# ExaScience/elprep

Measured on AMD Instinct MI355X. Metric: Mreads/s through sort+markdup+BQSR, 150bp PE, higher is better.
Workload: dtype u8/int32/int64 (integer path; float64 finalize on host)

## Files before the change

elprep_amd/csrc/common.hpp:

```cpp
#pragma once

#include <hip/hip_runtime.h>

#include <sched.h>

#include <cstdarg>
#include <cstdint>
#include <cstdio>
#include <cstring>
#include <map>
#include <mutex>
#include <string>
#include <vector>

#include "../../include/elprep_hip.h"
#include "../../include/elprep_hip_debug.h"
#include "derived.hpp"

namespace elp {

constexpr int WAVE = 64;

enum : uint16_t {
  F_MULTIPLE = 0x1, F_PROPER = 0x2, F_UNMAPPED = 0x4, F_NEXT_UNMAPPED = 0x8, F_REVERSED = 0x10, F_NEXT_REVERSED = 0x20,
// ... 116 lines not shown
  int tables_max_cycle = 0;
  unsigned long long tables_quals[2] = {0, 0};
  elp::DVec<unsigned long long> tables_pack;
  elp::DVec<uint8_t> lut_rows_dev;
  void *comm = nullptr;
  bool comm_borrowed = false;
  int (*xport)(void *, int64_t *, size_t) = nullptr;
  void *xport_user = nullptr;
  int (*p2p)(void *, int, const void *, size_t, int, void *, size_t) = nullptr;
  void *p2p_user = nullptr;
  int group_rank = 0, group_world = 1;
  elp_ctx *group_owner = nullptr;
  std::vector<elp_ctx *> group_borrowers;

  elp::DVec<uint8_t> raw;
  elp::DVec<uint64_t> raw_off;
  uint64_t raw_n = 0, raw_bytes = 0;
  uint64_t max_raw_rec = 0;
  elp::DVec<uint8_t> rg_ids;
  elp::DVec<uint32_t> rg_ids_off;
  bool have_rg_ids = false;
  static constexpr size_t TAG_WORDS = 65536 / 32;
  bool tag_filter = false;
  std::vector<uint32_t> h_tag_drop;
  elp::DVec<uint32_t> tag_drop;
  bool replace_rg = false;
  std::string replace_rg_id;
  elp::DVec<uint8_t> replace_rg_dev;
  hipStream_t copy_stream = nullptr;
  elp::DVec<uint8_t> lut_dev;
  void *lut_pinned = nullptr;
  size_t lut_pinned_cap = 0;
  hipEvent_t lut_ev = nullptr;
  hipEvent_t apply_ev = nullptr;
  int lut_uploaded_cycle = 0;
  elp::DVec<uint32_t> lut_wk;
  bool dict_ready = false;
  bool dict_per_cov = false;
  int dict_qlo = 0, dict_nqi = 0, dict_lmax = 0, dict_cycle = 0, dict_ncov = 0;
  hipEvent_t tables_ev = nullptr;
  void *bounce[2] = {nullptr, nullptr};
  hipEvent_t bounce_ev[2] = {nullptr, nullptr};

  uint32_t *mail = nullptr;
  hipEvent_t mail_ev = nullptr;

  elp_ctx *side[2] = {nullptr, nullptr};
  hipEvent_t side_ev[2] = {nullptr, nullptr};
  hipEvent_t side_done[2] = {nullptr, nullptr};
  bool sort_ahead = false;
  uint64_t presort_n = 0;
  uint64_t *presort_ks = nullptr;
  int presort_idx_bits = 0;

  elp::DVec<uint16_t> snap_flag;
  elp::DVec<uint8_t> snap_qual;
  uint64_t snap_n = 0, snap_qual_bytes = 0;

  struct Tuning {
    int count_kernel = 0;
    int apply_kernel = 0;
    int count3_rlog = -1;
    int qual_hint = 0;
    int qual_hint_drop = -1;
    int pair_table_slots = 1 << 20;
    long long bgzf_piece = 1ll << 30;
    int bgzf_weak_guess = 0;
    int score_kernel = 0;
    int mate_path = 0;
    int radix_tile = 0;
    int sort_pairs = 0;
    int tie_rounds = 0;
    int exchange_piece = 0;
    int emit_pass = 0;
    long long bgzf_inflate_piece = 2ll << 30;
    int bgzf_copy_chunk = 0;
    int bgzf_tok_lds = 0;
    int bgzf_first_chunk_div = 4;
    int bgzf_fixed = 0;
    int bgzf_tok_fail_above = 0;
    int bgzf_stored = 0;
    int apply_wgs = 0;
    int count3_grid = 0;
    int presort_tile = 0;
    int side_priority = 0;
  } tune;

  elp::DVec<uint8_t> scratch[8];

  bool profiling = false;
  const char *prof_prefix = nullptr;
  std::vector<std::string> prof_names;
  std::map<std::string, int> prof_index;
  std::vector<uint64_t> prof_launches;
  std::vector<double> prof_ms;
  std::vector<elp::ProfPending> prof_pending;
};

namespace elp {

int set_error(elp_ctx *c, int code, const char *fmt, ...);
int prof_begin(elp_ctx *c, const char *name);
void prof_end(elp_ctx *c, int pending);
int prof_flush(elp_ctx *c);
struct ProfScope {
  elp_ctx *c;
  const char *saved;
  ProfScope(elp_ctx *ctx, const char *prefix) : c(ctx), saved(ctx->prof_prefix) { ctx->prof_prefix = prefix; }
  ~ProfScope() { c->prof_prefix = saved; }
};

#define ELP_HIP(ctx, call)                                                                             \
  do {                                                                                                 \
    hipError_t e__ = (call);                                                                           \
    if (e__ != hipSuccess)                                                                             \
      return elp::set_error((ctx), e__ == hipErrorOutOfMemory ? ELP_ERR_NOMEM : ELP_ERR_HIP, "%s failed: %s (%s:%d)", #call, \
                            hipGetErrorString(e__), __FILE__, __LINE__);                               \
  } while (0)

#define ELP_TRY(expr)            \
  do {                           \
    int rc__ = (expr);           \
    if (rc__ != 0) return rc__;  \
  } while (0)

bool sync_spin();
inline void spin_relax(unsigned &spins) {
  if (++spins < 4096u) {
#if defined(__x86_64__) || defined(__i386__)
    __builtin_ia32_pause();
#elif defined(__aarch64__)
    asm volatile("yield");
#endif
  } else {
    sched_yield();
  }
}
inline hipError_t stream_wait(hipStream_t st) {
  if (!sync_spin()) return hipStreamSynchronize(st);
  hipError_t e;
  unsigned spins = 0;
  while ((e = hipStreamQuery(st)) == hipErrorNotReady) spin_relax(spins);
  return e;
}
inline hipError_t event_wait(hipEvent_t ev) {
  if (!sync_spin()) return hipEventSynchronize(ev);
  hipError_t e;
  unsigned spins = 0;
  while ((e = hipEventQuery(ev)) == hipErrorNotReady) spin_relax(spins);
  return e;
}

int debug_poison();
bool debug_trace();

template <class T>
int ensure(elp_ctx *c, DVec<T> &v, size_t n, bool keep = false, size_t keep_elems = 0) {
  if (n <= v.cap) return 0;
  size_t ncap = keep ? (n + n / 2 + 16) : n;
  T *np = nullptr;
  ELP_HIP(c, hipMalloc((void **)&np, ncap * sizeof(T) + debug_guard_bytes()));
  if (debug_guard_bytes()) debug_guard_arm(np, ncap * sizeof(T));
  if (const int pz = debug_poison(); pz >= 0) {
    ELP_HIP(c, hipMemsetAsync(np, pz, ncap * sizeof(T), c->stream));
    ELP_HIP(c, elp::stream_wait(c->stream));
  }
// ... 135 lines not shown
```

elprep_amd/csrc/ctx.hip:

```cpp
#include "common.hpp"

namespace elp {

namespace {
constexpr size_t GUARD = 4096;
constexpr uint8_t GUARD_BYTE = 0xC3;
std::mutex guard_mu;
std::map<void *, size_t> guard_of;
int guard_check_one(void *p, size_t payload) {
  uint8_t host[GUARD];
  if (hipDeviceSynchronize() != hipSuccess || hipMemcpy(host, static_cast<uint8_t *>(p) + payload, GUARD, hipMemcpyDeviceToHost) != hipSuccess) return 0;
  for (size_t k = 0; k < GUARD; k++)
    if (host[k] != GUARD_BYTE) {
      fprintf(stderr, "[elp] ELP_DEBUG_GUARD: byte %zu behind the end of a %zu-byte device buffer was overwritten (0x%02x)\n", k, payload, host[k]);
      return 1;
    }
  return 0;
}
}
size_t debug_guard_bytes() {
  static const size_t v = [] { const char *e = getenv("ELP_DEBUG_GUARD"); return (e && *e && *e != '0') ? GUARD : (size_t)0; }();
  return v;
}
void debug_guard_arm(void *p, size_t payload) {
// ... 513 lines not shown

int elp_get_permutation(elp_ctx *c, uint32_t *out) {
  if (!c || (!out && c->n)) return ELP_ERR_ARG;
  if (!c->derived.sorted) return set_error(c, ELP_ERR_ARG, "elp_get_permutation: call elp_sort_coordinate or elp_sort_queryname first");
  ELP_TRY(radix_check(c));
  return d2h(c, out, c->perm.p, c->n * sizeof(uint32_t));
}
int elp_get_flags(elp_ctx *c, uint16_t *out) {
  if (!c || (!out && c->n)) return ELP_ERR_ARG;
  ELP_TRY(radix_check(c));
  return d2h(c, out, c->flag.p, c->n * sizeof(uint16_t));
}
int elp_get_adapted(elp_ctx *c, int32_t *upos, int32_t *score) {
  if (!c) return ELP_ERR_ARG;
  ELP_TRY(ensure_adapted(c));
  if (upos) ELP_TRY(d2h(c, upos, c->upos.p, c->n * sizeof(int32_t)));
  if (score) ELP_TRY(d2h(c, score, c->score.p, c->n * sizeof(int32_t)));
  return 0;
}
int elp_get_qual(elp_ctx *c, uint8_t *out) {
  if (!c || (!out && c->qual_bytes)) return ELP_ERR_ARG;
  return d2h(c, out, c->qual.p, c->qual_bytes);
}

int elp_snapshot(elp_ctx *c) {
  if (!c) return ELP_ERR_ARG;
  ELP_HIP(c, hipSetDevice(c->device));
  ELP_TRY(ensure(c, c->snap_flag, c->n + 1));
  ELP_TRY(ensure(c, c->snap_qual, c->qual_bytes + 16));
  if (c->n) ELP_HIP(c, hipMemcpyAsync(c->snap_flag.p, c->flag.p, c->n * sizeof(uint16_t), hipMemcpyDeviceToDevice, c->stream));
  if (c->qual_bytes) ELP_HIP(c, hipMemcpyAsync(c->snap_qual.p, c->qual.p, c->qual_bytes, hipMemcpyDeviceToDevice, c->stream));
  c->snap_n = c->n;
  c->snap_qual_bytes = c->qual_bytes;
  c->derived.have_snapshot = true;
  return 0;
}
int elp_rollback(elp_ctx *c) {
  if (!c) return ELP_ERR_ARG;
  if (!c->derived.have_snapshot || c->snap_n != c->n || c->snap_qual_bytes != c->qual_bytes)
    return set_error(c, ELP_ERR_ARG, "elp_rollback: no snapshot of the current record set");
  ELP_HIP(c, hipSetDevice(c->device));
  if (c->n) ELP_HIP(c, hipMemcpyAsync(c->flag.p, c->snap_flag.p, c->n * sizeof(uint16_t), hipMemcpyDeviceToDevice, c->stream));
  if (c->qual_bytes) ELP_HIP(c, hipMemcpyAsync(c->qual.p, c->snap_qual.p, c->qual_bytes, hipMemcpyDeviceToDevice, c->stream));
  c->derived.flag_qual_restored();
  return 0;
}

int elp_set_tuning(elp_ctx *c, const char *key, int64_t value) {
  if (!c || !key) return ELP_ERR_ARG;
  const std::string k(key);
  const int v = (int)value;
  if (k == "count_kernel") c->tune.count_kernel = v;
  else if (k == "apply_kernel") c->tune.apply_kernel = v;
  else if (k == "bgzf_piece") { if (value < 1) return set_error(c, ELP_ERR_ARG, "elp_set_tuning: bgzf_piece must be positive"); c->tune.bgzf_piece = value; }
  else if (k == "bgzf_weak_guess") c->tune.bgzf_weak_guess = v;
  else if (k == "score_kernel") { c->tune.score_kernel = v; c->derived.score_tuning_changed(); }
  else if (k == "count3_rlog") c->tune.count3_rlog = v;
  else if (k == "qual_hint") { c->tune.qual_hint = v; c->derived.hint_tuning_changed(); }
  else if (k == "qual_hint_drop") { c->tune.qual_hint_drop = v; c->derived.hint_tuning_changed(); }
  else if (k == "pair_table_slots") {
    if (v == 0) { c->tune.pair_table_slots = 1 << 20; return 0; }
    if (v < 2 || v > (1 << 20) || (v & (v - 1))) return set_error(c, ELP_ERR_ARG, "elp_set_tuning: pair_table_slots must be a power of two >= 2");
    c->tune.pair_table_slots = v;
  } else if (k == "mate_path") {
    if (value != 0 && value != 2) return set_error(c, ELP_ERR_ARG, "elp_set_tuning: mate_path is 0 (the library decides) or 2 (every candidate through the table)");
    c->tune.mate_path = v;
  } else if (k == "tie_rounds") c->tune.tie_rounds = v;
  else if (k == "radix_tile") c->tune.radix_tile = v;
  else if (k == "sort_pairs") c->tune.sort_pairs = v;
  else if (k == "exchange_piece") c->tune.exchange_piece = v;
  else if (k == "emit_pass") c->tune.emit_pass = v;
  else if (k == "bgzf_stored") c->tune.bgzf_stored = v;
  else if (k == "bgzf_tok_fail_above") c->tune.bgzf_tok_fail_above = v;
  else if (k == "bgzf_fixed") c->tune.bgzf_fixed = v;
  else if (k == "bgzf_first_chunk_div") c->tune.bgzf_first_chunk_div = v;
  else if (k == "bgzf_tok_lds") c->tune.bgzf_tok_lds = v;
  else if (k == "bgzf_copy_chunk") c->tune.bgzf_copy_chunk = v;
  else if (k == "bgzf_inflate_piece") { if (value < 1) return set_error(c, ELP_ERR_ARG, "elp_set_tuning: bgzf_inflate_piece must be positive"); c->tune.bgzf_inflate_piece = value; }
  else if (k == "md_fused" || k == "bgzf_inflate") {
    if (value != 0) return set_error(c, ELP_ERR_ARG, "elp_set_tuning: key '%s' is retired (only 0 is accepted)", key);
  } else if (k == "apply_wgs") c->tune.apply_wgs = v;
  else if (k == "presort_tile") c->tune.presort_tile = v;
  else if (k == "count3_grid") { if (value < 0) return set_error(c, ELP_ERR_ARG, "elp_set_tuning: count3_grid must not be negative"); c->tune.count3_grid = v; }
  else if (k == "side_priority") c->tune.side_priority = v;
  else return set_error(c, ELP_ERR_ARG, "elp_set_tuning: unknown key '%s'", key);
  return 0;
}

int elp_profile_enable(elp_ctx *c, int on) {
  if (!c) return ELP_ERR_ARG;
  if (!on) { ELP_TRY(prof_flush(c)); prof_merge_side(c); }
  c->profiling = on != 0;
  for (int lane = 0; lane < 2; lane++)
    if (c->side[lane]) c->side[lane]->profiling = c->profiling;
  return 0;
}
int elp_profile_reset(elp_ctx *c) {
  if (!c) return ELP_ERR_ARG;
  ELP_TRY(prof_flush(c));
  prof_merge_side(c);
  for (auto &v : c->prof_launches) v = 0;
  for (auto &v : c->prof_ms) v = 0.0;
  return 0;
}
int elp_profile_count(elp_ctx *c) {
  if (!c) return ELP_ERR_ARG;
  if (prof_flush(c) != 0) return ELP_ERR_HIP;
  prof_merge_side(c);
  return (int)c->prof_names.size();
}
int elp_profile_get(elp_ctx *c, int index, const char **name, uint64_t *launches, double *total_ms) {
  if (!c || index < 0 || index >= (int)c->prof_names.size()) return ELP_ERR_ARG;
  if (name) *name = c->prof_names[index].c_str();
  if (launches) *launches = c->prof_launches[index];
  if (total_ms) *total_ms = c->prof_ms[index];
  return 0;
}

}
```

elprep_amd/csrc/markdup.hip:

```cpp
#include "common.hpp"

namespace elp {

constexpr uint32_t EMPTY = 0xFFFFFFFFu;
constexpr unsigned long long PB_EMPTY = ~0ull;

struct MdCols {
  uint64_t n;
  const int32_t *refid;
  const uint16_t *flag_in;
  const uint16_t *rgid;
  const uint16_t *rg_lib;
  const uint16_t *split;
  const int32_t *upos, *score;
  const uint64_t *qname_off;
  const uint8_t *qname;
};

__device__ __forceinline__ bool is_candidate(uint16_t f) { return (f & (F_UNMAPPED | F_SECONDARY | F_SUPPLEMENTARY)) == 0; }
__device__ __forceinline__ bool is_true_pair(uint16_t f) { return (f & (F_MULTIPLE | F_NEXT_UNMAPPED)) == F_MULTIPLE; }
__device__ __forceinline__ uint16_t lib_of(const MdCols &m, uint32_t i) {
  const uint16_t rg = m.rgid[i];
  return rg == ELP_NIL16 ? (uint16_t)ELP_NIL16 : m.rg_lib[rg];
}
__device__ __forceinline__ uint32_t ld_agent(const uint32_t *p) { return __hip_atomic_load(p, __ATOMIC_RELAXED, __HIP_MEMORY_SCOPE_AGENT); }
__device__ __forceinline__ unsigned long long ld_agent64(const unsigned long long *p) {
  return __hip_atomic_load(p, __ATOMIC_RELAXED, __HIP_MEMORY_SCOPE_AGENT);
}

__device__ __forceinline__ bool key_eq(const uint4 &a, const uint4 &b) { return a.x == b.x && a.y == b.y && a.z == b.z && a.w == b.w; }
__device__ __forceinline__ uint64_t frag_hash(const uint4 &k) {
  const uint64_t h = ((uint64_t)k.x << 32) | k.y;
  return mix64(mix64(h) ^ (((uint64_t)k.w << 32) | (uint64_t)k.z));
}

template <class Eq>
__device__ __forceinline__ uint32_t find_or_insert(uint32_t *table, uint64_t mask, uint64_t h, uint32_t i, Eq eq, uint64_t limit = ~0ull) {
  uint64_t s = h & mask;
  for (uint64_t probes = 0;; probes++) {
    if (probes > limit) return EMPTY;
    const uint32_t cur = atomicCAS(&table[s], EMPTY, i);
    if (cur == EMPTY) return i;
    if (cur == i || eq(cur, i)) return cur;
    s = (s + 1) & mask;
  }
}

__global__ __launch_bounds__(256) void k_frag_insert(MdCols m, const uint4 *__restrict__ fkey, const uint32_t *__restrict__ flist, uint32_t nf,
                                                     uint32_t *table, uint64_t mask, uint32_t *__restrict__ frep, unsigned long long *fbest) {
  const uint32_t j = blockIdx.x * blockDim.x + threadIdx.x;
  if (j >= nf) return;
  const uint32_t i = flist[j];
  const uint4 mine = fkey[i];
  const uint32_t rep = find_or_insert(table, mask, frag_hash(mine), i, [&](uint32_t a, uint32_t) { return key_eq(fkey[a], mine); });
  frep[i] = rep;
  atomicMax(&fbest[rep], (unsigned long long)(uint32_t)m.score[i]);
}
__global__ __launch_bounds__(256) void k_frag_bits(const uint32_t *__restrict__ table, uint64_t nwords, uint32_t *__restrict__ bits) {
  const uint64_t w = (uint64_t)blockIdx.x * blockDim.x + threadIdx.x;
  if (w >= nwords) return;
  const uint4 *t = reinterpret_cast<const uint4 *>(table + 32 * w);
  uint32_t b = 0;
#pragma unroll
  for (int k = 0; k < 8; k++) {
    const uint4 v = t[k];
    b |= (v.x != EMPTY ? 1u : 0u) << (4 * k) | (v.y != EMPTY ? 2u : 0u) << (4 * k) | (v.z != EMPTY ? 4u : 0u) << (4 * k) | (v.w != EMPTY ? 8u : 0u) << (4 * k);
  }
  bits[w] = b;
}
__device__ __forceinline__ void tournament(const MdCols &m, uint32_t *winner, uint32_t me) {
  uint32_t w = ld_agent(winner);
  for (;;) {
    if (w == EMPTY) {
      const uint32_t old = atomicCAS(winner, EMPTY, me);
      if (old == EMPTY) return;
      w = old;
      continue;
    }
    const int cq = qname_cmp(m.qname, m.qname_off, me, w);
    const bool better = cq < 0 || (cq == 0 && me > w);
    if (!better) return;
    const uint32_t old = atomicCAS(winner, w, me);
    if (old == w) return;
    w = old;
  }
}

__global__ __launch_bounds__(256) void k_frag_tie(MdCols m, const uint32_t *__restrict__ flist, uint32_t nf, const uint32_t *__restrict__ frep,
                                                  const unsigned long long *__restrict__ fbest, uint32_t *fwinner) {
  const uint32_t j = blockIdx.x * blockDim.x + threadIdx.x;
  if (j >= nf) return;
  const uint32_t i = flist[j];
  const uint32_t rep = frep[i];
  const unsigned long long b = fbest[rep];
  if ((b >> 63) || (unsigned long long)(uint32_t)m.score[i] != b) return;
  tournament(m, &fwinner[rep], (uint32_t)i);
}

__global__ __launch_bounds__(256) void k_frag_flag(MdCols m, const uint32_t *__restrict__ flist, uint32_t nf, const uint32_t *__restrict__ frep,
                                                   const unsigned long long *__restrict__ fbest, const uint32_t *__restrict__ fwinner,
                                                   uint16_t *__restrict__ flag_out) {
  const uint32_t j = blockIdx.x * blockDim.x + threadIdx.x;
  if (j >= nf) return;
  const uint32_t i = flist[j];
  const uint32_t rep = frep[i];
  const unsigned long long b = fbest[rep];
  const bool dup = (b >> 63) || (unsigned long long)(uint32_t)m.score[i] < b || fwinner[rep] != (uint32_t)i;
  if (dup) flag_out[i] = (uint16_t)(flag_out[i] | F_DUPLICATE);
}

struct PairKey { uint4 k1, k2; };
__device__ __forceinline__ PairKey pair_key(const uint4 &second, const uint4 &first) {
  const int32_t r1 = (int32_t)second.x, r2 = (int32_t)first.x, p1 = (int32_t)second.y, p2 = (int32_t)first.y;
  const bool v1 = second.z & 1u, v2 = first.z & 1u;
  const bool swap = r1 > r2 || (r1 == r2 && (p1 > p2 || (p1 == p2 && v1 && !v2)));
  return swap ? PairKey{first, second} : PairKey{second, first};
}
__device__ __forceinline__ bool pair_key_eq(const PairKey &a, const PairKey &b) {
  return a.k1.x == b.k1.x && a.k2.x == b.k2.x && a.k1.y == b.k1.y && a.k2.y == b.k2.y && a.k1.z == b.k1.z && ((a.k2.z ^ b.k2.z) & 1u) == 0 &&
         a.k1.w == b.k1.w;
}

__device__ __forceinline__ uint64_t pair_hash(const PairKey &k) {
  uint64_t h = mix64(((uint64_t)k.k1.x << 32) | k.k2.x);
  h = mix64(h ^ (((uint64_t)k.k1.y << 32) | k.k2.y));
  return mix64(h ^ (((uint64_t)k.k1.z << 1) | (k.k2.z & 1u)) ^ ((uint64_t)k.k1.w << 40));
}

__device__ __forceinline__ uint64_t qname_hash(const MdCols &m, uint32_t i) {
  const uint64_t o = m.qname_off[i];
  const uint32_t l = (uint32_t)(m.qname_off[i + 1] - o);
  uint64_t h = 0x9e3779b97f4a7c15ull ^ l;
  for (uint32_t k = 0; k < l; k += 8) h = (h ^ low_bytes(load8(m.qname + o + k), l - k)) * 0xff51afd7ed558ccdull + (h >> 29);
  return mix64(h ^ ((uint64_t)lib_of(m, i) << 48) ^ ((uint64_t)m.split[i] << 24));
}
__device__ __forceinline__ bool mate_key_eq(const MdCols &m, const uint4 *__restrict__ fkey, uint32_t a, const uint4 &kb, uint32_t b) {
  const uint4 ka = fkey[a];
  return (ka.z >> 1) == (kb.z >> 1) && ka.w == kb.w && qname_eq(m.qname, m.qname_off, a, b);
}
__device__ __forceinline__ bool is_mate_candidate(uint16_t f) { return is_candidate(f) && is_true_pair(f); }

enum : uint8_t { MC_NONE = 0, MC_TABLE = 1, MC_LEAD = 2, MC_FOLLOW = 3, MC_KIND = 3, MC_TABBED = 4  };
constexpr uint32_t MATE_BIG = 0xFFFFFFFEu;

__global__ __launch_bounds__(256) void k_bloom_coarse(const uint32_t *__restrict__ bloom, uint32_t n_lines, uint32_t *__restrict__ coarse) {
  const uint32_t line = blockIdx.x * 256 + threadIdx.x;
  bool nz = false;
  if (line < n_lines) {
    const uint4 *l = reinterpret_cast<const uint4 *>(bloom + (size_t)line * 16);
    const uint4 a = l[0], b = l[1], c2 = l[2], d = l[3];
    nz = (a.x | a.y | a.z | a.w | b.x | b.y | b.z | b.w | c2.x | c2.y | c2.z | c2.w | d.x | d.y | d.z | d.w) != 0;
// ... 419 lines not shown
  if ((f & (F_UNMAPPED | F_SECONDARY | F_SUPPLEMENTARY)) != 0) return 0;
  int32_t up = p;
  const uint64_t nop = c1 - c0;
  auto at = [&](uint64_t k) __attribute__((always_inline)) -> uint32_t { return k == 0 ? o0 : (k == 1 ? o1 : (k == 2 ? o2 : (k == 3 ? o3 : cigar[c0 + k]))); };
  if (nop) {
    if (f & F_REVERSED) {
      int32_t clipped = 1;
      up--;
      for (uint64_t k = nop; k-- > 0;) {
        const uint32_t c = at(k), op = c & 0xF;
        const int32_t isclip = (op == OP_S || op == OP_H) ? 1 : 0;
        const int32_t isref = op_consumes_ref(op) ? 1 : 0;
        clipped *= isclip;
        up += (isref | clipped) * (int32_t)(c >> 4);
      }
    } else {
      for (uint64_t k = 0; k < nop; k++) {
        const uint32_t c = at(k), op = c & 0xF;
        if (!(op == OP_S || op == OP_H)) break;
        up -= (int32_t)(c >> 4);
      }
    }
  }
  return up;
}
__device__ __forceinline__ uint16_t flag_in_of(uint16_t f, uint8_t state) { return state == 2 ? (uint16_t)(f | F_SECONDARY) : f; }

constexpr int FLI_CAP = 4096, FLI_CHUNK = 2048;
__global__ __launch_bounds__(256) void k_frag_list(FrontCols m, uint4 *__restrict__ fkey, uint32_t *__restrict__ flist, uint32_t *nf,
                                                   unsigned long long *__restrict__ fbest, uint32_t *__restrict__ fwinner) {
  __shared__ uint32_t lq[FLI_CAP];
  __shared__ uint32_t lcount, gbase;
  if (threadIdx.x == 0) lcount = 0;
  __syncthreads();
  const uint64_t nchunks = (m.n + FLI_CHUNK - 1) / FLI_CHUNK;
  for (uint64_t ch = blockIdx.x; ch < nchunks; ch += gridDim.x) {
    const uint64_t i0 = (ch * 256 + threadIdx.x) * 8;
    uint4 fv = make_uint4(0, 0, 0, 0);
    uint2 sv = make_uint2(0, 0);
    if (i0 < m.n) {
      fv = *reinterpret_cast<const uint4 *>(m.flag + i0);
      sv = *reinterpret_cast<const uint2 *>(m.state + i0);
    }
    const uint32_t fw[4] = {fv.x, fv.y, fv.z, fv.w};
    const uint64_t st8 = (uint64_t)sv.x | ((uint64_t)sv.y << 32);
    uint32_t fm = 0;
#pragma unroll
    for (int k = 0; k < 8; k++) {
      const uint16_t f = flag_in_of((uint16_t)(fw[k >> 1] >> (16 * (k & 1))), (uint8_t)(st8 >> (8 * k)));
      if (i0 + (uint64_t)k < m.n && is_candidate(f) && !is_true_pair(f)) fm |= 1u << k;
    }
    if (fm) {
      uint32_t at = atomicAdd(&lcount, (uint32_t)__popc(fm));
      for (; fm; fm &= fm - 1u) lq[at++] = (uint32_t)i0 + (uint32_t)(__ffs((int)fm) - 1);
    }
    __syncthreads();
    const uint32_t cnt = lcount;
    if (cnt + FLI_CHUNK <= (uint32_t)FLI_CAP && ch + gridDim.x < nchunks) continue;
    if (threadIdx.x == 0) gbase = cnt ? atomicAdd(nf, cnt) : 0u;
    __syncthreads();
    for (uint32_t k = threadIdx.x; k < cnt; k += 256) {
      const uint32_t i = lq[k];
      const uint16_t f = m.flag[i], rg = m.rgid[i];
      const uint64_t c0 = m.cigar_off[i], c1 = m.cigar_off[i + 1];
      const uint64_t nop = c1 - c0;
      const uint32_t o0 = nop > 0 ? m.cigar[c0] : 0u, o1 = nop > 1 ? m.cigar[c0 + 1] : 0u, o2 = nop > 2 ? m.cigar[c0 + 2] : 0u, o3 = nop > 3 ? m.cigar[c0 + 3] : 0u;
      const uint16_t lib = rg == ELP_NIL16 ? (uint16_t)ELP_NIL16 : m.rg_lib[rg];
      const int32_t up = unclipped_pos(f, m.pos[i], c0, c1, m.cigar, o0, o1, o2, o3);
      fkey[i] = make_uint4((uint32_t)m.refid[i], (uint32_t)up, ((uint32_t)lib << 1) | ((f & F_REVERSED) ? 1u : 0u), (uint32_t)m.split[i]);
      fbest[i] = 0;
      fwinner[i] = EMPTY;
      flist[gbase + k] = i;
    }
    __syncthreads();
    if (threadIdx.x == 0) lcount = 0;
    __syncthreads();
  }
}

constexpr int MF_THREADS = 320, MF_RECS = 312;
template <bool ADAPT>
__global__ __launch_bounds__(MF_THREADS) void k_md_front(FrontCols m, const int32_t *__restrict__ score, int32_t *__restrict__ upos_out, uint64_t *__restrict__ key_out,
                                                         uint4 *fkey, uint8_t *__restrict__ code, uint32_t *__restrict__ hash32, uint32_t *__restrict__ hash_lo, uint32_t *bloom,
                                                         uint32_t bloom_mask, uint32_t *n_table, const uint32_t *__restrict__ ftable, const uint32_t *__restrict__ fbits,
                                                         uint64_t fmask , unsigned long long *fbest, uint32_t *__restrict__ mate,
                                                         uint32_t *__restrict__ pair_win, uint64_t *__restrict__ pk, uint32_t *__restrict__ pv, uint32_t *np,
                                                         uint32_t nfixed, int optimistic) {
  const uint64_t base = (uint64_t)blockIdx.x * MF_RECS;
  const uint32_t t = threadIdx.x, lane = t & 63u, u = 63u * (t >> 6) + lane;
  const int64_t a_s = (int64_t)base - 2 + (int64_t)u;
  const bool own_rec = a_s >= 0 && (uint64_t)a_s < m.n;
  const bool valid = a_s >= 0 && (uint64_t)a_s + 1 < m.n;
  const uint64_t a = own_rec ? (uint64_t)a_s : 0;
  const uint16_t fa_st = m.flag[a], ra = m.rgid[a], sa = m.split[a];
  const uint8_t sta = m.state[a];
  const int32_t r = m.refid[a], p = m.pos[a], sc = score[a];
  const uint64_t oa = m.qname_off[a], oa1 = m.qname_off[a + 1];
  const uint64_t c0 = m.cigar_off[a], c1 = m.cigar_off[a + 1];
  const uint32_t la = (uint32_t)(oa1 - oa);
  const uint64_t nop = c1 - c0;
  const uint16_t lia = ra == ELP_NIL16 ? (uint16_t)ELP_NIL16 : m.rg_lib[ra];
  const uint8_t *pa = m.qname + oa;
  const uint64_t a0 = load8(pa), a1 = load8(pa + 8), a2 = load8(pa + 16), a3 = load8(pa + 24);
  const uint32_t o0 = nop > 0 ? m.cigar[c0] : 0u, o1 = nop > 1 ? m.cigar[c0 + 1] : 0u, o2 = nop > 2 ? m.cigar[c0 + 2] : 0u, o3 = nop > 3 ? m.cigar[c0 + 3] : 0u;
  const uint16_t fa = flag_in_of(fa_st, sta);
  const int32_t up = unclipped_pos(fa_st, p, c0, c1, m.cigar, o0, o1, o2, o3);
  const uint4 mine = make_uint4((uint32_t)r, (uint32_t)up, ((uint32_t)lia << 1) | ((fa & F_REVERSED) ? 1u : 0u), (uint32_t)sa);
  const uint64_t w0 = la > 0 ? low_bytes(a0, la) : 0ull, w1 = la > 8 ? low_bytes(a1, la - 8) : 0ull, w2 = la > 16 ? low_bytes(a2, la - 16) : 0ull,
                 w3 = la > 24 ? low_bytes(a3, la - 24) : 0ull;
  const uint32_t mcand = own_rec && is_mate_candidate(fa) ? 1u : 0u;
  const uint32_t nA = next_lane(mcand | ((uint32_t)lia << 1)), nL = next_lane(la);
  const uint32_t nS = next_lane((uint32_t)sa);
  const uint64_t b0 = next_lane64(w0), b1 = next_lane64(w1), b2 = next_lane64(w2), b3 = next_lane64(w3);
  const uint64_t n_oa = next_lane64(oa);
  bool join = valid && lane < 63u && mcand && (nA & 1u) && (uint16_t)(nA >> 1) == lia && (uint16_t)nS == sa && nL == la;
  if (join) {
    join = ((w0 ^ b0) | (w1 ^ b1) | (w2 ^ b2) | (w3 ^ b3)) == 0;
    const uint8_t *pb = m.qname + n_oa;
    for (uint32_t k = 32; join && k < la; k += 8) join = low_bytes(load8(pa + k), la - k) == low_bytes(load8(pb + k), la - k);
  }
  __shared__ uint8_t s_join[320];
  __shared__ uint4 s_fk[316];
  __shared__ int32_t s_sc[316];
  if (lane < 63u) {
    s_join[u] = join;
    s_fk[u] = mine;
    s_sc[u] = sc;
  }
  __syncthreads();
  const bool mine_rec = own_rec && lane < 63u && u >= 2u && u < 2u + (uint32_t)MF_RECS;
  const uint64_t i = a;
  uint8_t cd = MC_NONE;
  if (mine_rec) {
    if (ADAPT) {
      const uint64_t ru = sta ? (uint64_t)m.n_ref + 1 : (r < 0 ? (uint64_t)m.n_ref : (uint64_t)(uint32_t)r);
      key_out[i] = (ru << (m.pos_bits + 1)) | ((uint64_t)(uint32_t)p << 1) | ((fa_st & F_REVERSED) ? 1ull : 0ull);
      upos_out[i] = up;
    }
    if (!(is_candidate(fa) && !is_true_pair(fa))) fkey[i] = mine;
    pair_win[i] = EMPTY;
  }
  const uint8_t *j = s_join + u;
  if (mine_rec && mcand) {
    const bool nx = j[0], pv_ = j[-1];
    cd = MC_TABLE;
    if (nx && !pv_ && !j[1]) cd = MC_LEAD;
    else if (pv_ && !nx && !j[-2]) cd = MC_FOLLOW;
    if (cd != MC_FOLLOW) {
      uint64_t h = 0x9e3779b97f4a7c15ull ^ la;
      const uint64_t K = 0xff51afd7ed558ccdull;
      if (la > 0) h = (h ^ w0) * K + (h >> 29);
      if (la > 8) h = (h ^ w1) * K + (h >> 29);
      if (la > 16) h = (h ^ w2) * K + (h >> 29);
      if (la > 24) h = (h ^ w3) * K + (h >> 29);
      for (uint32_t k = 32; k < la; k += 8) h = (h ^ low_bytes(load8(pa + k), la - k)) * K + (h >> 29);
      h = mix64(h ^ ((uint64_t)lia << 48) ^ ((uint64_t)sa << 24));
      const uint32_t hi = (uint32_t)(h >> 32);
      hash32[i] = hi;
      if (cd == MC_TABLE) hash_lo[i] = (uint32_t)h;
      if (cd != MC_LEAD) atomicOr(&bloom[(hi >> 5) & bloom_mask], 1u << (hi & 31u));
    }
  }
  if (mine_rec) code[i] = cd;
  const unsigned long long tb = __ballot(cd == MC_TABLE);
  if (lane == 0 && tb) atomicAdd(&n_table[((blockIdx.x * 5u + (t >> 6)) & 63u) * 16u], (uint32_t)__popcll(tb));
  if (cd != MC_NONE && fmask) {
    uint64_t s = frag_hash(mine) & fmask;
    for (;; s = (s + 1) & fmask) {
      if (!((fbits[s >> 5] >> (s & 31)) & 1u)) break;
      const uint32_t c2 = ftable[s];
      if (key_eq(fkey[c2], mine)) {
        atomicMax(&fbest[c2], 1ull << 63);
        break;
      }
    }
  }
  if (mine_rec) mate[i] = !optimistic ? EMPTY : (cd == MC_LEAD ? (uint32_t)i + 1 : (cd == MC_FOLLOW ? (uint32_t)i - 1 : EMPTY));
  if (optimistic && mine_rec) {
    if (cd == MC_FOLLOW) {
      pk[i >> 1] = ((uint64_t)(uint32_t)(sc + s_sc[u - 1]) << 32) | (uint32_t)pair_hash(pair_key(mine, s_fk[u - 1]));
      pv[i >> 1] = (uint32_t)i;
    } else if (!(i & 1ull) && !(j[0] && !j[1] && !j[-1])) {
      pk[i >> 1] = 0xFFFFFFFF00000000ull | (uint32_t)mix64(i);
      pv[i >> 1] = EMPTY;
    }
    if (i == 0) *np = nfixed;
  }
}

static uint64_t table_size_for(uint64_t n) {
  uint64_t t = 1024;
  while (t < 2 * n + 16) t <<= 1;
  return t;
}

static int markdup_impl(elp_ctx *c) {
  const uint64_t n = c->n;
  ELP_TRY(ensure(c, c->mate, n + 1));
  ELP_TRY(ensure(c, c->pair_win, n + 1));
  if (n == 0) { ELP_TRY(ensure_adapted(c, true)); c->derived.marked = true; return 0; }
  const bool fuse_adapt = !c->derived.adapted();
  int pos_bits = 1;
  if (fuse_adapt) ELP_TRY(adapt_begin(c, &pos_bits));
  else ELP_TRY(ensure_adapted(c, false));
  const unsigned grid = blocks_for(n, 256);
  hipStream_t st = c->stream;
  MdCols m{n, c->refid.p, c->flag.p, c->rgid.p, c->rg_lib.p, c->split.p, c->upos.p, c->score.p, c->qname_off.p, c->qname.p};
  const uint64_t T = table_size_for(n);
  uint32_t *table;
  ELP_TRY(scratch(c, 0, T, &table));
  uint32_t *rep;
  unsigned long long *best;
  ELP_TRY(scratch(c, 2, n + 16, &best));
  uint32_t *winner;
  ELP_TRY(scratch(c, 3, n + 16, &winner));

  uint4 *fkey;
  ELP_TRY(scratch(c, 5, n + 8, &fkey));
  ELP_TRY(ensure(c, c->md_ctr, 16 + 64 * 16));
  uint32_t *nf_dev = c->md_ctr.p;
  ELP_TRY(scratch(c, 1, 2 * n + 16, &rep));
  uint32_t *flist = rep + n + 8;
  ELP_HIP(c, hipMemsetAsync(c->md_ctr.p, 0, (16 + 64 * 16) * sizeof(uint32_t), st));
  FrontCols fc{n, c->refid.p, c->pos.p, c->flag.p, c->has_sr.p, c->rgid.p, c->rg_lib.p, c->split.p, c->cigar_off.p, c->cigar.p, c->qname_off.p, c->qname.p,
               (uint32_t)c->n_ref, pos_bits};
  ELP_TRY(mailbox(c));
  ELP_LAUNCH(c, "md_frag_list", k_frag_list, dim3(std::min<unsigned>(blocks_for(n, FLI_CHUNK), (unsigned)c->n_cu * 8)), dim3(256), 0, fc, fkey, flist, nf_dev, best, winner);
  ELP_HIP(c, hipMemcpyAsync(c->mail, nf_dev, 4, hipMemcpyDeviceToHost, st));
  ELP_HIP(c, hipEventRecord(c->mail_ev, st));
  if (fuse_adapt) ELP_TRY(adapt_scores(c));

  int bbits = 0;
  while (bbits < 24 && ((n / 2 + 1) >> bbits) > (uint64_t)PB_TARGET) bbits++;
  const int ndig = (bbits + 7) / 8, sbits = 8 * ndig;
  const size_t nb = (size_t)1 << bbits;
  uint32_t *np_dev = c->md_ctr.p + 1;

  uint64_t bw = 1024;
  while (bw < n / 16 && bw < (1u << 20)) bw <<= 1;
  uint32_t *bloom, *hash32;
  uint8_t *code;
  const uint32_t tab_cap = (uint32_t)((blocks_for(n, 256 * MP_R) + 63) / 64) * 256u * MP_R;
  ELP_TRY(scratch(c, 6, bw + bw / 512 + 16 + n + 16 + (n + 16) / 4 + 64 * (size_t)tab_cap + 16 + n + 16, &bloom));
  uint32_t *coarse = bloom + bw;
  hash32 = coarse + bw / 512 + 16;
  code = reinterpret_cast<uint8_t *>(hash32 + n + 8);
  uint32_t *tab_list = hash32 + n + 16 + (n + 16) / 4;
  uint32_t *hash_lo = tab_list + 64 * (size_t)tab_cap + 8;
  uint32_t *rep_of = c->pair_win.p;
  uint32_t *n_table_dev = c->md_ctr.p + 16;
  ELP_HIP(c, hipMemsetAsync(bloom, 0, bw * sizeof(uint32_t), st));
  uint32_t n_tab = 0, n_tab64[64 * 16];
  uint32_t adapt_word[ADAPT_WORDS] = {0, 0, 0, 0, 0, 0};
  ELP_HIP(c, elp::event_wait(c->mail_ev));
  const uint32_t nf = c->mail[0];
  const unsigned fgrid = blocks_for(nf, 256);
  const uint64_t Tf = nf ? std::min<uint64_t>(T, table_size_for(4ull * nf)) : 0;
  const uint64_t npmax = n + 2;
  uint64_t *pk;
  ELP_TRY(scratch(c, 7, 2 * npmax + (2 * npmax + Tf + Tf / 32 + 64) / 2 + 8, &pk));
  uint32_t *pv = reinterpret_cast<uint32_t *>(pk + 2 * npmax), *ftable = pv + 2 * npmax, *fbits = ftable + Tf;
  if (nf) {
    ELP_HIP(c, hipMemsetAsync(ftable, 0xFF, Tf * sizeof(uint32_t), st));
    ELP_LAUNCH(c, "md_frag_insert", k_frag_insert, dim3(fgrid), dim3(256), 0, m, (const uint4 *)fkey, (const uint32_t *)flist, nf, ftable, Tf - 1, rep, best);
    ELP_LAUNCH(c, "md_frag_bits", k_frag_bits, dim3(blocks_for(Tf / 32, 256)), dim3(256), 0, (const uint32_t *)ftable, Tf / 32, fbits);
  }
  const int optimistic = c->tune.mate_path == 0;
  const uint32_t nfx = (uint32_t)((n + 1) / 2);
  if (fuse_adapt)
    ELP_LAUNCH(c, "md_front", k_md_front<true>, dim3(blocks_for(n, MF_RECS)), dim3(MF_THREADS), 0, fc, (const int32_t *)c->score.p, c->upos.p, c->key.p, fkey, code, hash32, hash_lo, bloom,
               (uint32_t)(bw - 1), n_table_dev, (const uint32_t *)ftable, (const uint32_t *)fbits, nf ? Tf - 1 : (uint64_t)0, best, c->mate.p, c->pair_win.p, pk, pv,
               np_dev, nfx, optimistic);
  else
    ELP_LAUNCH(c, "md_front", k_md_front<false>, dim3(blocks_for(n, MF_RECS)), dim3(MF_THREADS), 0, fc, (const int32_t *)c->score.p, c->upos.p, c->key.p, fkey, code, hash32, hash_lo, bloom,
               (uint32_t)(bw - 1), n_table_dev, (const uint32_t *)ftable, (const uint32_t *)fbits, nf ? Tf - 1 : (uint64_t)0, best, c->mate.p, c->pair_win.p, pk, pv,
               np_dev, nfx, optimistic);
  if (fuse_adapt) c->derived.keys = c->derived.scores = true;
  ELP_TRY(sort_presort(c));
  if (nf) {
    ELP_LAUNCH(c, "md_frag_tie", k_frag_tie, dim3(fgrid), dim3(256), 0, m, (const uint32_t *)flist, nf, (const uint32_t *)rep,
               (const unsigned long long *)best, winner);
    ELP_LAUNCH(c, "md_frag_flag", k_frag_flag, dim3(fgrid), dim3(256), 0, m, (const uint32_t *)flist, nf, (const uint32_t *)rep,
               (const unsigned long long *)best, (const uint32_t *)winner, c->flag.p);
  }
  ELP_HIP(c, hipMemcpyAsync(n_tab64, n_table_dev, sizeof n_tab64, hipMemcpyDeviceToHost, st));
  const bool adapt_read = c->derived.adapt_pending;
  if (adapt_read) ELP_HIP(c, hipMemcpyAsync(adapt_word, c->adapt_err.p, sizeof adapt_word, hipMemcpyDeviceToHost, st));
  ELP_HIP(c, elp::stream_wait(st));
  if (adapt_read) adapt_note(c, adapt_word);
  if (c->derived.adapt_bad_qual) return adapt_quality_error(c);
  for (int k = 0; k < 64; k++) n_tab += n_tab64[k * 16];

  const bool fixed = (uint64_t)n_tab < n / 8 && c->tune.mate_path == 0;
  const uint64_t nfixed = fixed ? (n + 1) / 2 : 0;
  const bool fast = fixed && n_tab == 0;
  if (!fast) ELP_HIP(c, hipMemsetAsync(c->mate.p, 0xFF, n * sizeof(uint32_t), st));
  if (n_tab && !fast) ELP_LAUNCH(c, "md_bloom_coarse", k_bloom_coarse, dim3(blocks_for(bw / 16, 256)), dim3(256), 0, (const uint32_t *)bloom, (uint32_t)(bw / 16), coarse);

  uint64_t Tm = fixed ? std::min<uint64_t>(T, table_size_for(std::min<uint64_t>(n, 4ull * n_tab + 1024))) : T;
  uint32_t e[4] = {0, 0, 0, 0};
  const bool listed = fixed && n_tab != 0;
  while (!fast) {
    ELP_HIP(c, hipMemsetAsync(table, 0xFF, Tm * sizeof(uint32_t), st));
    ELP_HIP(c, hipMemsetD32Async(reinterpret_cast<hipDeviceptr_t>(np_dev), (int)(uint32_t)nfixed, 1, st));
    if (listed) ELP_HIP(c, hipMemsetAsync(n_table_dev, 0, 64 * 16 * sizeof(uint32_t), st));
    ELP_LAUNCH(c, "md_mate_pairs", k_mate_pairs, dim3(blocks_for(n, 256 * MP_R)), dim3(256), 0, m, (const uint4 *)fkey, code,
               (const uint32_t *)hash32, (const uint32_t *)hash_lo, (const uint32_t *)bloom, (uint32_t)(bw - 1), (const uint32_t *)(n_tab ? coarse : nullptr), table, Tm - 1, c->mate.p,
               rep_of, c->err_flag.p, fixed ? 1 : 0, pk, pv, listed ? tab_list : (uint32_t *)nullptr, n_table_dev, tab_cap);
    if (listed)
      ELP_LAUNCH(c, "md_mate_table", k_mate_table, dim3(blocks_for(std::min<uint64_t>(n, 2ull * n_tab + 4096), 256)), dim3(256), 0, m, (const uint4 *)fkey, (const uint8_t *)code,
                 (const uint32_t *)hash32, (const uint32_t *)hash_lo, (const uint32_t *)tab_list, (const uint32_t *)n_table_dev, tab_cap, table, Tm - 1, c->mate.p, rep_of,
                 c->err_flag.p);
    ELP_TRY(fetch_err(c, e));
    if (!(e[1] & 2u)) break;
    if (Tm == T) return set_error(c, ELP_ERR_HIP, "mark duplicates: mate table overflow");
    Tm = T;
    ELP_HIP(c, hipMemsetAsync(c->err_flag.p + 1, 0, 4, st));
    ELP_HIP(c, hipMemsetAsync(c->mate.p, 0xFF, n * sizeof(uint32_t), st));
    ELP_HIP(c, hipMemsetAsync(rep_of, 0xFF, n * sizeof(uint32_t), st));
  }
  if (e[1]) {
    ELP_HIP(c, hipMemsetAsync(c->err_flag.p + 1, 0, 4, st));
    uint64_t *bk;
    uint32_t *bv, *cnt_dev = c->err_flag.p + 3;
    ELP_TRY(scratch(c, 2, 2 * n + 8, &bk));
    ELP_TRY(scratch(c, 3, 2 * n + 8, &bv));
    ELP_HIP(c, hipMemsetAsync(cnt_dev, 0, 4, st));
    ELP_LAUNCH(c, "md_big_collect", k_big_collect, dim3(grid), dim3(256), 0, n, (const uint32_t *)rep_of, c->mate.p, bk, bv, cnt_dev);
    uint32_t cnt = 0;
    ELP_HIP(c, hipMemcpyAsync(&cnt, cnt_dev, 4, hipMemcpyDeviceToHost, st));
    ELP_HIP(c, elp::stream_wait(st));
    ELP_HIP(c, hipMemsetAsync(cnt_dev, 0, 4, st));
    uint64_t *ks;
    uint32_t *vs;
    ProfScope ps(c, "md_big_");
    ELP_TRY(radix_sort_pairs(c, bk, bv, bk + n, bv + n, cnt, &ks, &vs));
    ELP_LAUNCH(c, "md_big_pair", k_big_pair, dim3(blocks_for(cnt, 256)), dim3(256), 0, cnt, (const uint64_t *)ks, c->mate.p);
  }

  {
    uint32_t *bounds;
    ELP_TRY(scratch(c, 1, 2 * nb + 8, &bounds));
    const bool folded = ndig > 0;
    ELP_HIP(c, hipMemsetAsync(bounds, folded ? 0xFF : 0, 2 * nb * sizeof(uint32_t), st));
    const bool no_table = fixed && n_tab == 0 && !e[1];
    if (!no_table) {
      ELP_HIP(c, hipMemsetAsync(c->pair_win.p, 0xFF, n * sizeof(uint32_t), st));
      if (listed)
        ELP_LAUNCH(c, "md_pair_list", k_pair_list_lists, dim3(blocks_for(std::min<uint64_t>(n, 2ull * n_tab + 4096), 256 * PL_TILES)), dim3(256), 0, m, (const uint4 *)fkey,
                   (const uint32_t *)c->mate.p, (const uint32_t *)tab_list, (const uint32_t *)n_table_dev, tab_cap, pk, pv, np_dev);
      else
        ELP_LAUNCH(c, "md_pair_list", k_pair_list_table, dim3(blocks_for(n, 256 * PL_TILES)), dim3(256), 0, m, (const uint4 *)fkey, (const uint32_t *)c->mate.p,
                   (const uint8_t *)code, pk, pv, np_dev);
    }
    uint64_t *ks = pk;
    uint32_t *vs = pv;
    if (ndig) {
      ProfScope ps(c, "md_pair_");
// ... 25 lines not shown
```

Measured before the change: 2333.

## Replace fragment occupancy bitmap with per-slot hash tag bytes for SIMD probing

The fragment hash table drops the separate occupancy-bitmap kernel. The insert kernel now writes a one-byte tag (high bit set plus hash bits) per occupied slot. In md_front, each lookup loads 16 tag bytes as a uint4, prefetched early, and matches them against the probe tag with SWAR byte compares. Only tag-matching slots dereference ftable and fkey. This saves one launch and cuts random key loads on probe misses, at the cost of a Tf-byte memset, a bit more register pressure in md_front, and a non-atomic tag write racing the CAS that still relies on kernel ordering.

New measurement: 2351 (median of 4 runs). No clear change (+0.8%).

```diff
diff --git a/elprep_amd/csrc/common.hpp b/elprep_amd/csrc/common.hpp
--- a/elprep_amd/csrc/common.hpp
+++ b/elprep_amd/csrc/common.hpp
@@ -222,6 +222,7 @@
     int bgzf_stored = 0;
     int apply_wgs = 0;
     int count3_grid = 0;
+    int frag_tag_bits = 0;
     int presort_tile = 0;
     int side_priority = 0;
   } tune;
diff --git a/elprep_amd/csrc/ctx.hip b/elprep_amd/csrc/ctx.hip
--- a/elprep_amd/csrc/ctx.hip
+++ b/elprep_amd/csrc/ctx.hip
@@ -619,6 +619,7 @@
   } else if (k == "apply_wgs") c->tune.apply_wgs = v;
   else if (k == "presort_tile") c->tune.presort_tile = v;
   else if (k == "count3_grid") { if (value < 0) return set_error(c, ELP_ERR_ARG, "elp_set_tuning: count3_grid must not be negative"); c->tune.count3_grid = v; }
+  else if (k == "frag_tag_bits") { if (value < 0 || value > 7) return set_error(c, ELP_ERR_ARG, "elp_set_tuning: frag_tag_bits is 0 (the default, 7) or 1 .. 7"); c->tune.frag_tag_bits = v; }
   else if (k == "side_priority") c->tune.side_priority = v;
   else return set_error(c, ELP_ERR_ARG, "elp_set_tuning: unknown key '%s'", key);
   return 0;
diff --git a/elprep_amd/csrc/markdup.hip b/elprep_amd/csrc/markdup.hip
--- a/elprep_amd/csrc/markdup.hip
+++ b/elprep_amd/csrc/markdup.hip
@@ -46,27 +46,34 @@
   }
 }
 
+__device__ __forceinline__ uint8_t frag_tag(uint64_t h, uint32_t tag_mask) { return (uint8_t)(0x80u | ((uint32_t)(h >> 56) & tag_mask)); }
+__device__ __forceinline__ uint64_t zero_bytes(uint64_t x) {
+  const uint64_t m = 0x7F7F7F7F7F7F7F7Full;
+  return ~(((x & m) + m) | x | m);
+}
 __global__ __launch_bounds__(256) void k_frag_insert(MdCols m, const uint4 *__restrict__ fkey, const uint32_t *__restrict__ flist, uint32_t nf,
-                                                     uint32_t *table, uint64_t mask, uint32_t *__restrict__ frep, unsigned long long *fbest) {
+                                                     uint32_t *table, uint64_t mask, uint8_t *__restrict__ ftag, uint32_t tag_mask, uint32_t *__restrict__ frep,
+                                                     unsigned long long *fbest) {
   const uint32_t j = blockIdx.x * blockDim.x + threadIdx.x;
   if (j >= nf) return;
   const uint32_t i = flist[j];
   const uint4 mine = fkey[i];
-  const uint32_t rep = find_or_insert(table, mask, frag_hash(mine), i, [&](uint32_t a, uint32_t) { return key_eq(fkey[a], mine); });
+  const uint64_t h = frag_hash(mine);
+  uint32_t rep;
+  for (uint64_t s = h & mask;; s = (s + 1) & mask) {
+    const uint32_t cur = atomicCAS(&table[s], EMPTY, i);
+    if (cur == EMPTY) {
+      ftag[s] = frag_tag(h, tag_mask);
+      rep = i;
+      break;
+    }
+    if (cur == i || key_eq(fkey[cur], mine)) {
+      rep = cur;
+      break;
+    }
+  }
   frep[i] = rep;
   atomicMax(&fbest[rep], (unsigned long long)(uint32_t)m.score[i]);
-}
-__global__ __launch_bounds__(256) void k_frag_bits(const uint32_t *__restrict__ table, uint64_t nwords, uint32_t *__restrict__ bits) {
-  const uint64_t w = (uint64_t)blockIdx.x * blockDim.x + threadIdx.x;
-  if (w >= nwords) return;
-  const uint4 *t = reinterpret_cast<const uint4 *>(table + 32 * w);
-  uint32_t b = 0;
-#pragma unroll
-  for (int k = 0; k < 8; k++) {
-    const uint4 v = t[k];
-    b |= (v.x != EMPTY ? 1u : 0u) << (4 * k) | (v.y != EMPTY ? 2u : 0u) << (4 * k) | (v.z != EMPTY ? 4u : 0u) << (4 * k) | (v.w != EMPTY ? 8u : 0u) << (4 * k);
-  }
-  bits[w] = b;
 }
 __device__ __forceinline__ void tournament(const MdCols &m, uint32_t *winner, uint32_t me) {
   uint32_t w = ld_agent(winner);
@@ -652,7 +659,7 @@
 template <bool ADAPT>
 __global__ __launch_bounds__(MF_THREADS) void k_md_front(FrontCols m, const int32_t *__restrict__ score, int32_t *__restrict__ upos_out, uint64_t *__restrict__ key_out,
                                                          uint4 *fkey, uint8_t *__restrict__ code, uint32_t *__restrict__ hash32, uint32_t *__restrict__ hash_lo, uint32_t *bloom,
-                                                         uint32_t bloom_mask, uint32_t *n_table, const uint32_t *__restrict__ ftable, const uint32_t *__restrict__ fbits,
+                                                         uint32_t bloom_mask, uint32_t *n_table, const uint32_t *__restrict__ ftable, const uint4 *__restrict__ ftag16, uint32_t tag_mask,
                                                          uint64_t fmask , unsigned long long *fbest, uint32_t *__restrict__ mate,
                                                          uint32_t *__restrict__ pair_win, uint64_t *__restrict__ pk, uint32_t *__restrict__ pv, uint32_t *np,
                                                          uint32_t nfixed, int optimistic) {
@@ -679,6 +686,10 @@
   const uint64_t w0 = la > 0 ? low_bytes(a0, la) : 0ull, w1 = la > 8 ? low_bytes(a1, la - 8) : 0ull, w2 = la > 16 ? low_bytes(a2, la - 16) : 0ull,
                  w3 = la > 24 ? low_bytes(a3, la - 24) : 0ull;
   const uint32_t mcand = own_rec && is_mate_candidate(fa) ? 1u : 0u;
+  const bool mine_rec = own_rec && lane < 63u && u >= 2u && u < 2u + (uint32_t)MF_RECS;
+  const bool look = mine_rec && mcand && fmask;
+  const uint64_t fh = frag_hash(mine);
+  const uint4 tg0 = look ? ftag16[(fh & fmask) >> 4] : make_uint4(0, 0, 0, 0);
   const uint32_t nA = next_lane(mcand | ((uint32_t)lia << 1)), nL = next_lane(la);
   const uint32_t nS = next_lane((uint32_t)sa);
   const uint64_t b0 = next_lane64(w0), b1 = next_lane64(w1), b2 = next_lane64(w2), b3 = next_lane64(w3);
@@ -698,7 +709,6 @@
     s_sc[u] = sc;
   }
   __syncthreads();
-  const bool mine_rec = own_rec && lane < 63u && u >= 2u && u < 2u + (uint32_t)MF_RECS;
   const uint64_t i = a;
   uint8_t cd = MC_NONE;
   if (mine_rec) {
@@ -734,15 +744,34 @@
   if (mine_rec) code[i] = cd;
   const unsigned long long tb = __ballot(cd == MC_TABLE);
   if (lane == 0 && tb) atomicAdd(&n_table[((blockIdx.x * 5u + (t >> 6)) & 63u) * 16u], (uint32_t)__popcll(tb));
-  if (cd != MC_NONE && fmask) {
-    uint64_t s = frag_hash(mine) & fmask;
-    for (;; s = (s + 1) & fmask) {
-      if (!((fbits[s >> 5] >> (s & 31)) & 1u)) break;
-      const uint32_t c2 = ftable[s];
-      if (key_eq(fkey[c2], mine)) {
-        atomicMax(&fbest[c2], 1ull << 63);
-        break;
+  if (look) {
+    uint64_t g = (fh & fmask) >> 4;
+    uint32_t b = (uint32_t)fh & 15u;
+    uint4 tg = tg0;
+    const uint64_t pat = 0x0101010101010101ull * frag_tag(fh, tag_mask);
+    for (;;) {
+      const uint64_t lo = (uint64_t)tg.x | ((uint64_t)tg.y << 32), hi = (uint64_t)tg.z | ((uint64_t)tg.w << 32);
+      const uint64_t klo = b < 8u ? ~0ull << (8u * b) : 0ull, khi = b <= 8u ? ~0ull : ~0ull << (8u * (b - 8u));
+      const uint64_t elo = ~lo & 0x8080808080808080ull & klo, ehi = ~hi & 0x8080808080808080ull & khi;
+      uint64_t mlo = zero_bytes(lo ^ pat) & klo, mhi = zero_bytes(hi ^ pat) & khi;
+      const uint32_t pe = elo ? (uint32_t)__builtin_ctzll(elo) >> 3 : (ehi ? 8u + ((uint32_t)__builtin_ctzll(ehi) >> 3) : 16u);
+      bool found = false;
+      while (mlo | mhi) {
+        const uint32_t k = mlo ? (uint32_t)__builtin_ctzll(mlo) >> 3 : 8u + ((uint32_t)__builtin_ctzll(mhi) >> 3);
+        if (k >= pe) break;
+        if (mlo) mlo &= mlo - 1ull;
+        else mhi &= mhi - 1ull;
+        const uint32_t c2 = ftable[(g << 4) + k];
+        if (key_eq(fkey[c2], mine)) {
+          atomicMax(&fbest[c2], 1ull << 63);
+          found = true;
+          break;
+        }
       }
+      if (found || pe < 16u) break;
+      g = (g + 1) & (fmask >> 4);
+      b = 0;
+      tg = ftag16[g];
     }
   }
   if (mine_rec) mate[i] = !optimistic ? EMPTY : (cd == MC_LEAD ? (uint32_t)i + 1 : (cd == MC_FOLLOW ? (uint32_t)i - 1 : EMPTY));
@@ -828,22 +857,24 @@
   const uint64_t Tf = nf ? std::min<uint64_t>(T, table_size_for(4ull * nf)) : 0;
   const uint64_t npmax = n + 2;
   uint64_t *pk;
-  ELP_TRY(scratch(c, 7, 2 * npmax + (2 * npmax + Tf + Tf / 32 + 64) / 2 + 8, &pk));
-  uint32_t *pv = reinterpret_cast<uint32_t *>(pk + 2 * npmax), *ftable = pv + 2 * npmax, *fbits = ftable + Tf;
+  ELP_TRY(scratch(c, 7, 2 * npmax + (2 * npmax + Tf + Tf / 4 + 64) / 2 + 8, &pk));
+  uint32_t *pv = reinterpret_cast<uint32_t *>(pk + 2 * npmax), *ftable = pv + 2 * npmax;
+  uint8_t *ftag = reinterpret_cast<uint8_t *>((reinterpret_cast<uintptr_t>(ftable + Tf) + 15) & ~(uintptr_t)15);
+  const uint32_t tag_mask = (1u << (c->tune.frag_tag_bits > 0 ? c->tune.frag_tag_bits : 7)) - 1u;
   if (nf) {
     ELP_HIP(c, hipMemsetAsync(ftable, 0xFF, Tf * sizeof(uint32_t), st));
-    ELP_LAUNCH(c, "md_frag_insert", k_frag_insert, dim3(fgrid), dim3(256), 0, m, (const uint4 *)fkey, (const uint32_t *)flist, nf, ftable, Tf - 1, rep, best);
-    ELP_LAUNCH(c, "md_frag_bits", k_frag_bits, dim3(blocks_for(Tf / 32, 256)), dim3(256), 0, (const uint32_t *)ftable, Tf / 32, fbits);
+    ELP_HIP(c, hipMemsetAsync(ftag, 0, Tf, st));
+    ELP_LAUNCH(c, "md_frag_insert", k_frag_insert, dim3(fgrid), dim3(256), 0, m, (const uint4 *)fkey, (const uint32_t *)flist, nf, ftable, Tf - 1, ftag, tag_mask, rep, best);
   }
   const int optimistic = c->tune.mate_path == 0;
   const uint32_t nfx = (uint32_t)((n + 1) / 2);
   if (fuse_adapt)
     ELP_LAUNCH(c, "md_front", k_md_front<true>, dim3(blocks_for(n, MF_RECS)), dim3(MF_THREADS), 0, fc, (const int32_t *)c->score.p, c->upos.p, c->key.p, fkey, code, hash32, hash_lo, bloom,
-               (uint32_t)(bw - 1), n_table_dev, (const uint32_t *)ftable, (const uint32_t *)fbits, nf ? Tf - 1 : (uint64_t)0, best, c->mate.p, c->pair_win.p, pk, pv,
+               (uint32_t)(bw - 1), n_table_dev, (const uint32_t *)ftable, (const uint4 *)ftag, tag_mask, nf ? Tf - 1 : (uint64_t)0, best, c->mate.p, c->pair_win.p, pk, pv,
                np_dev, nfx, optimistic);
   else
     ELP_LAUNCH(c, "md_front", k_md_front<false>, dim3(blocks_for(n, MF_RECS)), dim3(MF_THREADS), 0, fc, (const int32_t *)c->score.p, c->upos.p, c->key.p, fkey, code, hash32, hash_lo, bloom,
-               (uint32_t)(bw - 1), n_table_dev, (const uint32_t *)ftable, (const uint32_t *)fbits, nf ? Tf - 1 : (uint64_t)0, best, c->mate.p, c->pair_win.p, pk, pv,
+               (uint32_t)(bw - 1), n_table_dev, (const uint32_t *)ftable, (const uint4 *)ftag, tag_mask, nf ? Tf - 1 : (uint64_t)0, best, c->mate.p, c->pair_win.p, pk, pv,
                np_dev, nfx, optimistic);
   if (fuse_adapt) c->derived.keys = c->derived.scores = true;
   ELP_TRY(sort_presort(c));
```
